# python-graphblas/python-graphblas

Measured on AMD Instinct MI355X. Metric: GTEPS (mxv) on R-MAT scale-24, higher is better.
Workload: dtype f32

## Files before the change

include/grb_mi355x.h:

```cpp
#ifndef GRB_MI355X_H
#define GRB_MI355X_H

#include <stdbool.h>
#include <stddef.h>
#include <stdint.h>

#ifdef __cplusplus
extern "C" {
#endif

#define GRB_VERSION 2
#define GRB_SUBVERSION 0

typedef uint64_t GrB_Index;
#define GrB_INDEX_MAX ((GrB_Index)(1ULL << 60) - 1)

typedef enum {
    GrB_SUCCESS = 0,
    GrB_NO_VALUE = 1,
    GrB_UNINITIALIZED_OBJECT = -1,
    GrB_NULL_POINTER = -2,
    GrB_INVALID_VALUE = -3,
    GrB_INVALID_INDEX = -4,
    GrB_DOMAIN_MISMATCH = -5,
// ... 192 lines not shown
    int64_t flops;
    int64_t out_nvals;
    int32_t method;
    int32_t fused_epilogue;
    int64_t hot_k;
    int64_t long_entries;
    int64_t long_segments;
    int32_t long_kernel;
    int32_t reorders;
    int64_t ordered;
    int64_t value_dict;
    int64_t fill_absent;
    int64_t long_probe;
    int64_t long_tails;
    int64_t pinned_natural;
} GrX_Stats;
GrB_Info GrX_last_stats(GrX_Stats *stats);
GrB_Info GrX_mxm_streamed(const GrB_Semiring semiring, const GrB_Matrix A, const GrB_Matrix B, uint64_t budget_bytes,
                          uint64_t *nvals, uint64_t *checksum, uint64_t *flops, uint64_t *batches);
GrB_Info GrX_Matrix_isclose(bool *result, const GrB_Matrix A, const GrB_Matrix B, double rel_tol, double abs_tol);
GrB_Info GrX_Matrix_dup_as(GrB_Matrix *C, const GrB_Type type, const GrB_Matrix A);
GrB_Info GrX_Vector_dup_as(GrB_Vector *w, const GrB_Type type, const GrB_Vector u);
GrB_Info GrX_Vector_fill_absent(GrB_Vector v, const GrB_Monoid monoid);
GrB_Info GrX_Matrix_cache_bytes(const GrB_Matrix A, uint64_t *bytes);
GrB_Info GrX_option_set(const char *name, int64_t value);
GrB_Info GrX_option_get(const char *name, int64_t *value);
GrB_Info GrX_options_reset(void);
const char *GrX_version_string(void);

#define GRB_DECL_UNARY(T)                                                                                              \
// ... 89 lines not shown
```

python-graphblas_amd/_lib.py:

```python
from __future__ import annotations

import ctypes
import os

_HERE = os.path.dirname(os.path.abspath(__file__))
DEFAULT_LIB = os.path.join(_HERE, "csrc", "libgrb_mi355x.so")

lib = None
_handles = {}

c_void_p = ctypes.c_void_p
c_u64 = ctypes.c_uint64
c_int = ctypes.c_int

TYPE_NAMES = ["BOOL", "INT8", "INT16", "INT32", "INT64", "UINT8", "UINT16", "UINT32", "UINT64", "FP32", "FP64"]

GrB_SUCCESS = 0
GrB_NO_VALUE = 1


class GrX_Stats(ctypes.Structure):
    _fields_ = [("kernel_launches", ctypes.c_int64), ("tiles", ctypes.c_int64), ("flops", ctypes.c_int64),
                ("out_nvals", ctypes.c_int64), ("method", ctypes.c_int32), ("fused_epilogue", ctypes.c_int32),
                ("hot_k", ctypes.c_int64), ("long_entries", ctypes.c_int64), ("long_segments", ctypes.c_int64),
                ("long_kernel", ctypes.c_int32), ("reorders", ctypes.c_int32), ("ordered", ctypes.c_int64), ("value_dict", ctypes.c_int64), ("fill_absent", ctypes.c_int64),
                ("long_probe", ctypes.c_int64), ("long_tails", ctypes.c_int64), ("pinned_natural", ctypes.c_int64)]


def load(path: str | None = None):
    global lib
    if lib is not None:
        return lib
    path = path or os.environ.get("GRB_MI355X_LIB") or DEFAULT_LIB
    if not os.path.exists(path):
        raise ImportError(
            f"{path} not found: build it with `python -c 'import __graft_entry__ as g; g.build()'` "
            "(there is no pure-Python or CPU fallback)"
        )
    if os.path.basename(path) == os.path.basename(DEFAULT_LIB):
        _share_hip_runtime_with_torch()
    lib = ctypes.CDLL(path)
# ... 151 lines not shown
```

python-graphblas_amd/csrc/grb_context.hip:

```cpp
#include <chrono>
#include <algorithm>
#include <cctype>
#include <cstdlib>
#include <cstring>
#include <mutex>
#include <unordered_map>
#include <vector>

#include "grb_internal.hpp"

namespace grb {

#ifdef GRB_ABLATE
static constexpr int DEBUG_FLAGS_MASK = ~0;
#else
static constexpr int DEBUG_FLAGS_MASK = 128 | 256 | 2048 | 65536;
#endif


Context &ctx()
{
    static Context c;
    return c;
}
// ... 183 lines not shown
    int Context::*i;
    int64_t Context::*l;
    enum Rule { ANY, WITHIN, ONE_OF, CLAMP } rule;
    int64_t lo, hi;
    bool (*hook)(int64_t &value);
};
using Hook = bool (*)(int64_t &);
constexpr int64_t MAX64 = INT64_MAX, P30 = 1 << 30;
constexpr Option opt(const char *n, int Context::*f, Option::Rule r = Option::ANY, int64_t lo = 0, int64_t hi = 0, Hook h = nullptr) { return {n, f, nullptr, r, lo, hi, h}; }
constexpr Option opt(const char *n, int64_t Context::*f, Option::Rule r = Option::ANY, int64_t lo = 0, int64_t hi = 0, Hook h = nullptr) { return {n, nullptr, f, r, lo, hi, h}; }

bool known_debug_flags(int64_t &v) { return !((int)v & ~DEBUG_FLAGS_MASK); }
bool short_kernel_exists(int64_t &v) { return v != 2 && v != 3 && v != 4; }
bool snap_long_classes(int64_t &v) { if (v != 16 && v != 32 && v != 64) v = 8; return true; }
bool window_group(int64_t &v) { return (v & (v - 1)) == 0; }
bool release_cache_when_off(int64_t &v) { if (!v) dev_cache_release(); return true; }

const Option OPTIONS[] = {
    opt("debug_flags", &Context::debug_flags, Option::ANY, 0, 0, known_debug_flags),
    opt("pull_ipt", &Context::tune_pull_ipt),
    opt("hot_min_cols", &Context::hot_min_cols),
    opt("hot_k", &Context::hot_k),
    opt("push_mode", &Context::push_mode),
    opt("split_min_nnz", &Context::split_min_nnz),
    opt("split_min_len", &Context::split_min_len, Option::CLAMP, 0, P30),
    opt("short_kernel", &Context::short_kernel, Option::WITHIN, 0, 6, short_kernel_exists),
    opt("lazy_layout", &Context::lazy_layout),
    opt("lazy_min_nnz", &Context::lazy_min_nnz),
    opt("lean_min_nnz", &Context::lean_min_nnz, Option::CLAMP, 0, MAX64),
    opt("long_kernel", &Context::long_kernel),
// ... 10 lines not shown
    opt("mxm_unit_small", &Context::mxm_unit_small, Option::WITHIN, 1, P30),
    opt("mxm_unit_mid", &Context::mxm_unit_mid, Option::WITHIN, 1, P30),
    opt("mxm_unit_dense", &Context::mxm_unit_dense, Option::WITHIN, 1, P30),
    opt("mxm_sym_windows", &Context::mxm_sym_windows, Option::WITHIN, 1, 64),
    opt("mxm_window_groups", &Context::mxm_window_groups, Option::WITHIN, 0, 8, window_group),
    opt("mxm_xcd_map", &Context::mxm_xcd_map, Option::WITHIN, 0, 1),
    opt("mxm_checksum_pass", &Context::mxm_checksum_pass, Option::WITHIN, 0, 1),
    opt("mxm_bitmap_pool_mb", &Context::mxm_bitmap_pool_mb),
    opt("mxm_bitmap_min_cnt", &Context::mxm_bitmap_min_cnt),
    opt("mxm_bitmap_pool_cap", &Context::mxm_bitmap_pool_cap),
    opt("vec_pad_min_bytes", &Context::vec_pad_min_bytes),
    opt("hub_min_len", &Context::hub_min_len, Option::CLAMP, 0, P30),
    opt("fill_absent", &Context::fill_absent, Option::WITHIN, 0, 1),
    opt("rows_tile", &Context::rows_tile, Option::WITHIN, 0, 2),
    opt("lazy_tagged", &Context::lazy_tagged, Option::WITHIN, 0, 1),
    opt("ctile_pack", &Context::ctile_pack, Option::WITHIN, 0, 2),
    opt("strip_slot16", &Context::strip_slot16, Option::WITHIN, 0, 1),
    opt("rtile_pack", &Context::rtile_pack, Option::WITHIN, 0, 1),
    opt("cold_in_rows", &Context::cold_in_rows, Option::CLAMP, 0, P30),
    opt("stream_nt_min_nnz", &Context::stream_nt_min_nnz, Option::CLAMP, 0, MAX64),
    opt("bool_probe", &Context::bool_probe, Option::WITHIN, 0, 16),
    opt("rtile_rows", &Context::rtile_rows, Option::ONE_OF, 8192, 16384),
    opt("rtile_entries", &Context::rtile_entries, Option::WITHIN, 256, 1 << 24),
    opt("rows_head", &Context::rows_head, Option::WITHIN, 0, 1),
    opt("rows_head_min_groups", &Context::rows_head_min_groups, Option::CLAMP, 0, MAX64),
    opt("push_small", &Context::push_small, Option::WITHIN, 0, 1),
    opt("value_dict", &Context::value_dict, Option::WITHIN, 0, 1),
    opt("order_mode", &Context::order_mode, Option::WITHIN, 0, 1),
    opt("order_min_nnz", &Context::order_min_nnz, Option::CLAMP, 0, MAX64),
    opt("alloc_cache", &Context::alloc_cache, Option::ANY, 0, 0, release_cache_when_off),
};
// ... 211 lines not shown
```

python-graphblas_amd/csrc/grb_internal.hpp:

```cpp
#pragma once
#include <hip/hip_runtime.h>

#include <cstdint>
#include <cstdio>
#include <cstring>
#include <memory>
#include <string>
#include <type_traits>

#include "grb_mi355x.h"

namespace grb {

enum TypeCode : int {
    TC_BOOL = 0, TC_INT8, TC_INT16, TC_INT32, TC_INT64, TC_UINT8, TC_UINT16, TC_UINT32, TC_UINT64, TC_FP32, TC_FP64,
    TC_COUNT
};

enum OpCode : int {
    OP_NONE = -1,
    OP_FIRST = 0, OP_SECOND, OP_PAIR, OP_PLUS, OP_MINUS, OP_RMINUS, OP_TIMES, OP_MIN, OP_MAX,
    OP_LOR, OP_LAND, OP_LXOR, OP_LXNOR, OP_ANY, OP_COUNT,
    OP_EQ = 32, OP_NE, OP_GT, OP_LT, OP_GE, OP_LE,
    OP_UNSUPPORTED = 1000
// ... 80 lines not shown
    int rows_head = 1;
    int64_t rows_head_min_groups = 16384;
    int push_small = 1;
    int fill_absent = 1;
    int hub_min_len = 1024;
    int value_dict = 1;
    int order_mode = 1;
    int64_t order_min_nnz = 24ll << 20;
    int64_t reorder_count = 0;
    void *host_stage = nullptr;
    bool host_stage_failed = false;
    void *host_pinned = nullptr;
    unsigned long long *push_counters = nullptr;
    int push_parity = 0;
    int lazy_tagged = 1;
    int ctile_pack = 0;
    int strip_slot16 = 1;
    int rtile_pack = 1;
    int cold_in_rows = 0;
};
Context &ctx();
void require_init();

void *dev_alloc(size_t bytes);
void *dev_alloc_zero(size_t bytes);
void dev_free(void *p);
void dev_cache_release();
void h2d(void *dst, const void *src, size_t bytes);
void d2h(void *dst, const void *src, size_t bytes);
void d2d(void *dst, const void *src, size_t bytes);
// ... 394 lines not shown
```

python-graphblas_amd/csrc/grb_mxv.hip:

```cpp
#include <algorithm>
#include <cstring>
#include <vector>

#include "grb_internal.hpp"
#include "grb_ops.hpp"

namespace grb {

#include "grb_mxv_common.inc"
#include "grb_mxv_pull.inc"
#include "grb_mxv_long.inc"
#include "grb_mxv_vdict.inc"
#include "grb_mxv_strip.inc"
#include "grb_mxv_rows.inc"
#include "grb_mxv_rows_tag.inc"
#include "grb_mxv_ctile.inc"
#include "grb_mxv_rtile.inc"
#include "grb_mxv_split_build.inc"
#include "grb_mxv_write.inc"
#include "grb_mxv_push.inc"
#include "grb_mxv_hot.inc"
#include "grb_mxv_order.inc"

static int64_t hot_table_size(int64_t n, size_t value_bytes)
// ... 276 lines not shown
                               sub, sub_min_len, (unsigned)ncls, kind == 2 ? 1 : 0, 0u, (const int32_t *)nullptr, 0, (int64_t)0, 0u, 0u, (int64_t)0, 0u, (const int64_t *)nullptr);
            const int nvc = ncls + hub_ncls;
            const int n_cr = own_ranges ? A->order.ct_ncr : COLD_CLS * (int)sub;
            const int nvirt = kind == 4 ? nvc + n_cr + (tail_max > 0 ? 1 : 0) : ncls * (int)sub;
            const int hot_cls = 0;
            const unsigned strip_sub = kind == 4 ? 1u : sub;
            if (strips) {
                int vbits = 1;
                while ((1 << vbits) < nvirt) vbits++;
                prim_sort_pairs_u64_u32_bits(keys.p, keys2.p, idx.p, idx2.p, nnz_keyed, 32, 32 + vbits);
            } else {
                prim_sort_pairs_u64_u32(keys.p, keys2.p, idx.p, idx2.p, nnz_keyed, bits);
            }
            int ct_mode = 0;
            std::vector<int32_t> h_bounds;
            if (kind == 4 && own_ranges && ctx().ctile_pack > 0) {
                h_bounds.resize((size_t)A->order.ct_ncr + 1);
                d2h(h_bounds.data(), A->order.d_cold_bounds, sizeof(int32_t) * h_bounds.size());
                int64_t widest = 0;
                for (int r = 0; r < A->order.ct_ncr; r++) widest = std::max<int64_t>(widest, (int64_t)h_bounds[(size_t)r + 1] - (int64_t)h_bounds[(size_t)r]);
                if (widest < ((int64_t)1 << 19) - 1) ct_mode = (ctx().ctile_pack == 2 && A->vd.vdict_n > 0 && A->type->size == 4 && !A->iso) ? 2 : 1;
            }
            const int ct_slots = ct_mode ? CT_PACK_SLOTS : (A->type->size > 4 ? CT_SLOTS / 2 : CT_SLOTS);
            const int n_sb = (int)ceil_div(nl, (int64_t)ct_slots);
            const int64_t n_tiles = kind == 4 ? (int64_t)n_cr * n_sb : 0;
            std::vector<int64_t> h_first((size_t)n_tiles + 1, 0);
            DevBuf<int64_t> tile_first(n_tiles + 1);
            int64_t n_strip = nnz_long;
            if (kind == 4) {
                hipLaunchKernelGGL(k_ctile_first, dim3((unsigned)ceil_div(n_tiles + 1, 256)), dim3(256), 0, ctx().stream, (const uint64_t *)keys2.p, nnz_keyed,
                                   n_tiles, n_sb, (unsigned)nvc, tile_first.p, ct_slots);
                d2h(h_first.data(), tile_first.p, sizeof(int64_t) * (size_t)(n_tiles + 1));
                n_strip = h_first[0];
                if (h_first[(size_t)n_tiles] != nnz_long)
                    fail(GrB_PANIC, "long / short split: the short part and the class keys disagree about the cold entries that moved (internal error)");
            }
            if (kind == 4) {
                sp.long_nnz = nnz_long;
// ... 137 lines not shown
                        sp.strips.d_strip_cb.reset((int64_t *)dev_alloc(sizeof(int64_t) * (size_t)(nvc + 1)));
                        h2d(sp.strips.d_strip_cb, h_cb, sizeof(int64_t) * (size_t)(nvc + 1));
                        sp.strips.wg_tab_g = G;
                    }
                    if (getenv("GRB_PRINT_STRIPS")) {
                        fprintf(stderr, "[strips kind %d] %d classes (%d of them the hub level's), chunks per class:", kind, nvc, hub_ncls);
                        for (int c = 0; c < nvc; c++) fprintf(stderr, " %lld", (long long)(h_cb[c + 1] - h_cb[c]));
                        fprintf(stderr, "  segments %lld\n", (long long)nseg);
                    }
                    sp.strips.strip_ncls = ncls;
                    sp.strips.strip_nseg = nseg;
                    sp.long_nnz = nnz_long;
                    sync_stream();
                }
            }
            const bool use_dict_all = ct_mode == 2;
            if (kind == 4 && nnz_long > n_strip) {
                std::vector<CTile> h_tiles;
                std::vector<int64_t> h_efirst;
                std::vector<int> tile_range;
                std::vector<int64_t> range_cnt((size_t)n_cr, 0);
                int64_t units = 0;
                for (int64_t t = 0; t < n_tiles; t++) {
                    const int64_t cnt = h_first[t + 1] - h_first[t];
                    if (cnt == 0) continue;
                    const int64_t pieces = ceil_div(cnt, CT_MAX_ENTRIES), per = ceil_div(cnt, pieces);
                    for (int64_t q = 0; q < pieces; q++) {
                        const int64_t e0 = h_first[t] + q * per, e1 = std::min<int64_t>(h_first[t] + (q + 1) * per, h_first[t + 1]);
                        CTile ct;
                        ct.u0 = units;
                        ct.n_units = (int32_t)ceil_div(e1 - e0, (int64_t)CT_EPL);
// ... 22 lines not shown
                    }
                } else {
                    for (int r = 0; r < n_cr; r++) range_xcd[(size_t)r] = r % 8;
                }
                std::vector<int32_t> h_order;
                h_order.reserve((size_t)nt);
                for (int x = 0; x < 8; x++) {
                    sp.cold.ct_xoff[x] = (int64_t)h_order.size();
                    for (int64_t t = 0; t < nt; t++)
                        if (range_xcd[(size_t)tile_range[(size_t)t]] == x) h_order.push_back((int32_t)t);
                }
                sp.cold.ct_xoff[8] = (int64_t)h_order.size();
                const size_t ents = (size_t)std::max<int64_t>(units, 1) * CT_EPL;
                sp.cold.d_ct_tiles.reset(dev_alloc((sizeof(CTile) + sizeof(int32_t)) * (size_t)std::max<int64_t>(nt, 1)));
                h2d(sp.cold.d_ct_tiles, h_tiles.data(), sizeof(CTile) * (size_t)nt);
                if (ct_mode) {
                    std::vector<int32_t> h_cbase((size_t)nt);
                    for (int64_t t = 0; t < nt; t++) h_cbase[(size_t)t] = h_bounds[(size_t)tile_range[(size_t)t]];
                    h2d((char *)sp.cold.d_ct_tiles.get() + sizeof(CTile) * (size_t)std::max<int64_t>(nt, 1), h_cbase.data(), sizeof(int32_t) * (size_t)nt);
                }
                sp.cold.d_ct_order.reset((int32_t *)dev_alloc(sizeof(int32_t) * (size_t)std::max<int64_t>(nt, 1)));
                h2d(sp.cold.d_ct_order, h_order.data(), sizeof(int32_t) * (size_t)nt);
                DevBuf<int64_t> efirst(nt + 1);
                h2d(efirst.p, h_efirst.data(), sizeof(int64_t) * (size_t)(nt + 1));
                sp.cold.d_ct_col.reset((int32_t *)dev_alloc(sizeof(int32_t) * ents));
                const size_t ct_vb = use_dict_all ? 1 : A->type->size;
                sp.cold.d_ct_val.reset(A->iso ? nullptr : dev_alloc(ct_vb * ents));
                sp.cold.d_ct_loc.reset(ct_mode ? nullptr : (uint16_t *)dev_alloc(sizeof(uint16_t) * ents));
                GRB_HIP(hipMemsetAsync(sp.cold.d_ct_col, 0xff, sizeof(int32_t) * ents, ctx().stream));
                if (sp.cold.d_ct_val) GRB_HIP(hipMemsetAsync(sp.cold.d_ct_val, 0, ct_vb * ents, ctx().stream));
                if (sp.cold.d_ct_loc) GRB_HIP(hipMemsetAsync(sp.cold.d_ct_loc, 0, sizeof(uint16_t) * ents, ctx().stream));
                const int64_t n_cold = nnz_long - n_strip;
                {
                    DevBuf<uint64_t> key2(n_cold), key2s(n_cold);
                    DevBuf<uint32_t> pay(n_cold), pays(n_cold);
                    hipLaunchKernelGGL(k_ctile_keys2, dim3((unsigned)ceil_div(n_cold, 256)), dim3(256), 0, ctx().stream, (const uint32_t *)idx2.p, n_strip, n_cold,
                                       (const int64_t *)efirst.p, nt, col_src, key2.p, pay.p);
                    int tbits = 1;
                    while (((int64_t)1 << tbits) < nt) tbits++;
                    prim_sort_pairs_u64_u32(key2.p, key2s.p, pay.p, pays.p, n_cold, 32 + tbits);
                    GRB_DISPATCH_TYPE(A->type->code, T, {
                        hipLaunchKernelGGL((k_ctile_place<T>), dim3((unsigned)ceil_div(n_cold, 256)), dim3(256), 0, ctx().stream, (const uint64_t *)keys2.p,
                                           (const uint32_t *)idx2.p, n_strip, n_cold, (const uint64_t *)key2s.p, (const uint32_t *)pays.p, (const int64_t *)efirst.p,
                                           (const CTile *)sp.cold.d_ct_tiles.get(), (const T *)A->d_val, A->iso ? 1 : 0, sp.cold.d_ct_col, (T *)sp.cold.d_ct_val.get(), sp.cold.d_ct_loc,
                                           use_dict_all ? (const unsigned long long *)A->vd.d_vd_table : (const unsigned long long *)nullptr,
                                           use_dict_all ? (const unsigned char *)A->vd.d_vd_codes : (const unsigned char *)nullptr,
                                           ct_mode ? (const int32_t *)((const char *)sp.cold.d_ct_tiles.get() + sizeof(CTile) * (size_t)std::max<int64_t>(nt, 1)) : (const int32_t *)nullptr);
                    })
                    sync_stream();
                }
                sp.cold.ct_mode = ct_mode;
                sp.cold.ct_ntiles = nt;
                sp.cold.ct_units = units;
                if (getenv("GRB_PRINT_STRIPS")) {
                    fprintf(stderr, "[cold tiles] mode %d (slots %d), %d column ranges, %lld tiles, entries per range:", ct_mode, ct_slots, n_cr, (long long)nt);
                    for (int r = 0; r < n_cr; r++) fprintf(stderr, " %lld(x%d)", (long long)range_cnt[(size_t)r], range_xcd[(size_t)r]);
                    fprintf(stderr, "\n");
                }
                sync_stream();
            }
            DevBuf<int64_t> vptr(strips ? 0 : nv + 1), icnt(strips ? 0 : nv + 1);
            if (!strips) {
// ... 67 lines not shown
        if (A->hot_identity) {
            dev_free(A->d_col);
            A->d_col = nullptr;
        } else {
            A->hot.d_col_hot.reset();
        }
        A->hot.hot_cols_dropped = true;
    }
}

static uint64_t order_signature()
{
    const Context &c = ctx();
    uint64_t h = 1469598103934665603ull;
    const int64_t v[] = {c.long_kernel, c.short_kernel, c.long_classes, c.split_min_len, c.long_sub, c.long_sub_min_len, c.lean_min_nnz,
                         c.split_min_nnz, c.hot_k, c.drop_hot_cols, c.hub_min_len, c.value_dict, c.rows_tile, c.rtile_rows, c.rtile_entries, c.cold_in_rows, c.rtile_pack, c.strip_slot16, c.ctile_pack, c.lazy_tagged};
    for (int64_t x : v) h = (h ^ (uint64_t)x) * 1099511628211ull;
    return h;
}

static GB_Perm *ensure_perm(GB_Matrix_opaque *S, int64_t k_hot, DevBuf<unsigned int> &poscnt)
{
    const int64_t n = (int64_t)S->ncols, nnz = S->nvals;
    GB_Matrix_opaque *partner = S->tr ? S->tr : S->tr_of;
    const bool adopt = !S->order.perm && partner && partner->order.perm;
    if (adopt) {
        S->order.perm = partner->order.perm;
        perm_retain(S->order.perm);
    }
    DevBuf<unsigned int> cnt(n, true);
    const int hstride = nnz >= ((int64_t)1 << 26) ? 8 : 1;
// ... 410 lines not shown
            for (int c = 0; c <= A->split.strips.strip_ncls; c++) a.strip_cb[c] = A->split.strips.strip_cb[c];
            a.strip_ncls = A->split.strips.strip_ncls;
            const int64_t G = std::max<int64_t>(A->split.strips.strip_ncls, (int64_t)(ctx().num_cus / A->split.strips.strip_ncls) * A->split.strips.strip_ncls);
            if (A->split.split_kind == 4) {
                a.hrec = A->split.strips.d_hrec;
                a.hrec_bytes = A->split.strips.hrec_bytes;
                a.vdict = A->vd.vdict_n > 0 ? A->vd.d_vdict.get() : nullptr;
                ctx().stats.value_dict = A->vd.vdict_n;
                auto launch_ctile = [&]() {
                    if (A->split.cold.ct_units <= 0) return;
                    a.ct_col = A->split.cold.d_ct_col;
                    a.ct_val = A->split.cold.d_ct_val;
                    a.ct_loc = A->split.cold.d_ct_loc;
                    a.ct_tiles = (const CTile *)A->split.cold.d_ct_tiles.get();
                    a.ct_mode = A->split.cold.ct_mode;
                    a.ct_cbase = A->split.cold.ct_mode ? (const int32_t *)((const char *)A->split.cold.d_ct_tiles.get() + sizeof(CTile) * (size_t)std::max<int64_t>(A->split.cold.ct_ntiles, 1)) : nullptr;
                    if (A->split.cold.ct_mode == 2) a.vdict = A->vd.d_vdict;
                    a.ct_order = A->split.cold.d_ct_order;
                    for (int x = 0; x <= 8; x++) a.ct_xoff[x] = A->split.cold.ct_xoff[x];
                    const int64_t Gt = std::max<int64_t>(8, (int64_t)(ctx().num_cus * CT_WGS_PER_CU / 8) * 8);
                    hipLaunchKernelGGL((k_mxv_ctile<T, MON, MUL>), dim3((unsigned)Gt), dim3(CT_BLOCK), 0, ctx().stream, a);
                    ctx().stats.kernel_launches += 1;
                };
                bool merged = false;
                if constexpr (MON >= 0) {
                    if constexpr (hstrip_fast_semiring<T>(MON, MUL)) {
                        if (hot_fast && A->split.strips.hub_ncls > 0 && A->split.strips.d_wg_tab && A->split.strips.wg_tab_g > 0 && A->split.strips.strip_cb[A->split.strips.strip_ncls + A->split.strips.hub_ncls] > 0) {
                            PullArgs al = a;
                            al.wg_tab = A->split.strips.d_wg_tab;
                            al.strip_cb_dev = A->split.strips.d_strip_cb;
                            al.strip_chunks = A->split.strips.strip_cb[A->split.strips.strip_ncls + A->split.strips.hub_ncls];
                            bool dict_launched = false;
                            const bool s16 = al.strip_slot16 != nullptr;
                            if constexpr (sizeof(T) == 4) {
                                if (al.vdict) {
// ... 282 lines not shown
    DescFlags f;
    if (d) { f.replace = d->replace; f.comp = d->comp; f.structure = d->structure; f.t0 = d->t0; f.t1 = d->t1; }
    return f;
}

static void mxv_core(GB_Vector_opaque *w, GB_Vector_opaque *mask, const GB_BinaryOp_opaque *accum,
                     const GB_Semiring_opaque *sr, GB_Matrix_opaque *S, GB_Vector_opaque *u, bool flip, DescFlags f)
{
    if (S->ncols != u->n) fail(GrB_DIMENSION_MISMATCH, "mxv/vxm: matrix inner dimension " + std::to_string(S->ncols) + " does not match vector size " + std::to_string(u->n));
    if (w->n != S->nrows) fail(GrB_DIMENSION_MISMATCH, "mxv/vxm: output size " + std::to_string(w->n) + " does not match matrix dimension " + std::to_string(S->nrows));
    if (mask && mask->n != w->n) fail(GrB_DIMENSION_MISMATCH, "mxv/vxm: mask size does not match output size");
    if (accum && (accum->type != w->type->code || op_is_comparison(accum->op))) fail(GrB_DOMAIN_MISMATCH, "mxv/vxm: accum operator type must equal the output type");
    ctx().stats = GrX_Stats{};
    ctx().stats.method = 1;
    ctx().stats.long_kernel = -1;
    ctx().stats.flops = S->nvals;
    ctx().stats.out_nvals = -1;
    const int64_t m = (int64_t)w->n;
    if (m == 0) return;
    if (!mask && f.comp) {
        if (f.replace) vector_release_storage(w);
        return;
    }
    const int st = sr->type;
    const int monoid = canonical_op(st, sr->monoid);
    int mult = canonical_op(st, sr->mult);
    if (flip) mult = flip_op(mult);

    DevBuf<uint64_t> mbits_tmp(0);
    const uint64_t *m_bits = nullptr;
// ... 367 lines not shown
    const int need_u = !(mult == OP_PAIR || mult == OP_SECOND);
    if ((need_a && P->type->code != st) || (need_u && u->type->code != st) || w->type->code != st) return -1;
    if (u->n > 0xffffffffull || w->n > 0x7fffffffull || !u->d_val) return -1;
    const int64_t n_in = (int64_t)u->n, n_out = (int64_t)w->n;
    if (ctx().push_mode == 1 && u->nvals >= 0 && u->nvals * 64 >= n_in) return 0;
    if (ctx().push_mode == 1 && u->nvals >= 0 && n_in > 0 && (double)u->nvals * ((double)P->nvals / (double)n_in) * 128.0 > (double)P->nvals) return 0;
    GB_Vector_opaque *vs[3] = {u, w, mask};
    GB_Perm *ord = (u->n == w->n) ? vectors_common_order(vs, 3) : nullptr;
    if (u->n != w->n)
        for (GB_Vector_opaque *v : vs)
            if (v) vector_set_order(v, nullptr);
    ctx().stats = GrX_Stats{};
    ctx().stats.method = 2;
    ctx().stats.out_nvals = -1;
    ctx().stats.long_kernel = -1;
    PushThin a{};
    a.u_bits = u->d_bits;
    a.n_in = n_in;
    a.n_out = n_out;
    a.in_map = ord ? ord->d_inv : nullptr;
    a.out_map = ord ? ord->d_rank : nullptr;
    a.rowptr = matrix_rowptr(P);
    a.col = P->d_col;
    a.aval = P->d_val;
    a.a_iso = P->iso ? 1 : 0;
    a.u_val = u->d_val;
    a.monoid = monoid;
    a.mult = mult;
    a.need_a = need_a;
    a.need_u = need_u;
// ... 370 lines not shown
```

python-graphblas_amd/csrc/grb_mxv_ctile.inc:

```
#ifndef GRB_CT_SLOTS
#define GRB_CT_SLOTS 16384
#endif
#ifndef GRB_CT_BLOCK
#define GRB_CT_BLOCK 1024
#endif
constexpr int CT_SLOTS = GRB_CT_SLOTS;
constexpr int CT_PACK_SLOTS = 8192, CT_PACK_COLBITS = 19;
constexpr int CT_BLOCK = GRB_CT_BLOCK;
constexpr int CT_EPL = 4;
#ifndef GRB_CT_WGS_PER_CU
#define GRB_CT_WGS_PER_CU 2
#endif
constexpr int CT_WGS_PER_CU = GRB_CT_WGS_PER_CU;
#ifndef GRB_CT_ABL
#define GRB_CT_ABL 0
#endif
struct alignas(16) CTile {
    int64_t u0;
    int32_t n_units;
    int32_t base;
};
template <typename W> struct CtSlots { static constexpr int value = sizeof(W) > 4 ? CT_SLOTS / 2 : CT_SLOTS; };

#ifndef GRB_CT_MAX_ENTRIES
// ... 19 lines not shown
    const int64_t c = (int64_t)blockIdx.x * blockDim.x + threadIdx.x;
    if (c >= n_cold) return;
    const int64_t p = p0 + c;
    int64_t lo = 0, hi = n_tiles;
    while (hi - lo > 1) {
        const int64_t mid = (lo + hi) >> 1;
        if (efirst[mid] <= p) lo = mid;
        else hi = mid;
    }
    key2[c] = ((uint64_t)lo << 32) | (uint64_t)(uint32_t)col[sidx[p]];
    pay[c] = (uint32_t)c;
}
template <typename T>
__global__ void k_ctile_place(const uint64_t *skeys, const uint32_t *sidx, int64_t p0, int64_t n_cold, const uint64_t *key2s, const uint32_t *pays,
                              const int64_t *efirst, const CTile *tiles, const T *val, int iso, int32_t *tcol, T *tval, uint16_t *tloc,
                              const unsigned long long *vd_table, const unsigned char *vd_codes, const int32_t *cbase)
{
    const int64_t q = (int64_t)blockIdx.x * blockDim.x + threadIdx.x;
    if (q >= n_cold) return;
    const uint64_t k2 = key2s[q];
    const int64_t t = (int64_t)(k2 >> 32);
    const int64_t p = p0 + (int64_t)pays[q];
    const int64_t slot = (int64_t)(uint32_t)skeys[p];
    const int64_t d = tiles[t].u0 * CT_EPL + (q - (efirst[t] - p0));
    if (cbase) tcol[d] = (int32_t)((((uint32_t)(slot - tiles[t].base)) << CT_PACK_COLBITS) | (((uint32_t)k2 - (uint32_t)cbase[t]) & ((1u << CT_PACK_COLBITS) - 1u)));
    else tcol[d] = (int32_t)(uint32_t)k2;
    bool coded = false;
    if constexpr (sizeof(T) == 4) {
        if (vd_table) {
            ((unsigned char *)tval)[d] = (unsigned char)vdict_code(vd_table, vd_codes, ((const uint32_t *)val)[sidx[p]]);
            coded = true;
        }
    }
    if (!iso && !coded) tval[d] = val[sidx[p]];
    if (tloc) tloc[d] = (uint16_t)(slot - tiles[t].base);
}

template <typename T, int MONOID_CT, int MULT_CT>
__global__ __launch_bounds__(CT_BLOCK) void k_mxv_ctile(const PullArgs a)
{
    using W = typename Widen<T>::type;
    constexpr int EPL = CT_EPL, SLOTS = CtSlots<W>::value;
    __shared__ W s_acc[SLOTS];
    __shared__ uint32_t s_off[SLOTS / 32];
    __shared__ uint32_t s_has[SLOTS / 32];
    __shared__ uint32_t s_dict[sizeof(T) == 4 ? 256 : 1];
    const int monoid = MONOID_CT >= 0 ? MONOID_CT : a.monoid;
    const int mult = MULT_CT >= 0 ? MULT_CT : a.mult;
    const bool need_aval = a.need_aval != 0, need_uval = a.need_uval != 0;
    const bool stage_vals = need_aval && !a.a_iso;
    const bool snt = a.stream_nt != 0;
    const T iso_v = (a.a_iso && need_aval) ? ((const T *)a.aval)[0] : (T)0;
    const __amdgpu_buffer_rsrc_t xval_rs = make_rsrc(a.u_val, a.x_len * (int64_t)sizeof(T));
    const __amdgpu_buffer_rsrc_t xbits_rs = make_rsrc(a.u_bits, a.u_full ? 0 : ((a.x_len + 63) >> 6) * 8);
    const __amdgpu_buffer_rsrc_t xvbits_rs = make_rsrc(a.u_valbits, a.u_valbits ? ((a.x_len + 63) >> 6) * 8 : 0);
    const __amdgpu_buffer_rsrc_t xpv_rs = make_rsrc(a.u_pv, a.u_pv ? ((a.x_len + 15) >> 4) * 4 : 0);
    const int32_t *tcol = a.ct_col;
    const T *tval = (const T *)a.ct_val;
    const uint16_t *tloc = a.ct_loc;
    W *tl = (W *)a.tl_val;
    const W ident = pull_seed<T, W>(a, monoid);
    const int packed = a.ct_mode;
    const int slots_rt = packed ? (CT_PACK_SLOTS < SLOTS ? CT_PACK_SLOTS : SLOTS) : SLOTS;
    if constexpr (sizeof(T) == 4) {
        if (packed == 2) {
            for (int i = threadIdx.x; i < 256; i += CT_BLOCK) s_dict[i] = ((const uint32_t *)a.vdict)[i];
            __syncthreads();
        }
    }
    const int xcd = (int)(blockIdx.x & 7u), li = (int)(blockIdx.x >> 3), nx = (int)(gridDim.x >> 3);
    const int64_t x0 = a.ct_xoff[xcd], x1 = a.ct_xoff[xcd + 1];
    for (int64_t tl_i = x0 + li; tl_i < x1; tl_i += nx) {
        const CTile tile = a.ct_tiles[a.ct_order[tl_i]];
        if (tile.n_units == 0) continue;
        const int cbase = packed ? a.ct_cbase[a.ct_order[tl_i]] : 0;
        const int rows_here = (int)((a.n_long - tile.base < slots_rt) ? a.n_long - tile.base : slots_rt);
        for (int i = threadIdx.x; i < slots_rt; i += CT_BLOCK) s_acc[i] = ident;
        for (int i = threadIdx.x; i < slots_rt / 32; i += CT_BLOCK) {
            s_has[i] = 0u;
            const int64_t wd = ((int64_t)tile.base >> 5) + i;
            s_off[i] = (a.has_mask && (int64_t)i * 32 < rows_here) ? ~a.long_act[wd] : 0u;
        }
        __syncthreads();
        const int64_t u_end = tile.u0 + tile.n_units;
        constexpr int UB = 1;
        for (int64_t ub0 = tile.u0; ub0 < u_end; ub0 += (int64_t)CT_BLOCK * UB) {
            const int64_t ub = ub0 + threadIdx.x;
            int creg[UB][EPL], rk[UB][EPL], cc[UB][EPL];
            T vreg[UB][EPL];
            bool uv[UB];
#pragma unroll
            for (int k = 0; k < UB; k++) {
                const int64_t u = ub + (int64_t)k * CT_BLOCK;
                uv[k] = u < u_end;
                const int64_t e = (uv[k] ? u : u_end - 1) * EPL;
                const uint4 c4 = ptr_stream_x4(tcol + e, snt);
                creg[k][0] = (int)c4.x; creg[k][1] = (int)c4.y; creg[k][2] = (int)c4.z; creg[k][3] = (int)c4.w;
                if (packed) {
#pragma unroll
                    for (int i = 0; i < EPL; i++) {
                        const unsigned w = (unsigned)creg[k][i];
                        rk[k][i] = (int)(w >> CT_PACK_COLBITS);
                        creg[k][i] = w == 0xffffffffu ? -1 : cbase + (int)(w & ((1u << CT_PACK_COLBITS) - 1u));
                        if (w == 0xffffffffu) rk[k][i] = 0;
                    }
                } else {
                    const uint2 l2 = ptr_stream_x2(tloc + e, snt);
                    rk[k][0] = (int)(l2.x & 0xffffu); rk[k][1] = (int)(l2.x >> 16); rk[k][2] = (int)(l2.y & 0xffffu); rk[k][3] = (int)(l2.y >> 16);
                }
                bool vals_done = false;
                if constexpr (sizeof(T) == 4) {
                    if (stage_vals && packed == 2) {
                        const uint32_t cd = ((const uint32_t *)tval)[uv[k] ? u : u_end - 1];
#pragma unroll
                        for (int i = 0; i < EPL; i++) vreg[k][i] = __builtin_bit_cast(T, s_dict[(cd >> (8 * i)) & 0xffu]);
                        vals_done = true;
                    }
                }
                if (vals_done) {
                } else if (stage_vals) {
                    if constexpr (sizeof(T) == 4) {
                        const uint4 v4 = ptr_stream_x4(tval + e, snt);
                        vreg[k][0] = __builtin_bit_cast(T, v4.x); vreg[k][1] = __builtin_bit_cast(T, v4.y);
                        vreg[k][2] = __builtin_bit_cast(T, v4.z); vreg[k][3] = __builtin_bit_cast(T, v4.w);
                    } else {
#pragma unroll
// ... 52 lines not shown
#pragma unroll
                    for (int k = 0; k < UB; k++)
#pragma unroll
                        for (int i = 0; i < EPL; i++) xv[k][i] = vreg[k][i];
                } else {
#pragma unroll
                    for (int k = 0; k < UB; k++)
#pragma unroll
                        for (int i = 0; i < EPL; i++) xv[k][i] = buf_gather<T>(xval_rs, xp[k][i] ? (unsigned)cc[k][i] * (unsigned)sizeof(T) : 0xfffffff8u);
                }
            } else {
#pragma unroll
                for (int k = 0; k < UB; k++)
#pragma unroll
                    for (int i = 0; i < EPL; i++) xv[k][i] = (T)0;
            }
#pragma unroll
            for (int k = 0; k < UB; k++)
#pragma unroll
                for (int i = 0; i < EPL; i++) {
                    if (!xp[k][i]) continue;
                    const int r = rk[k][i];
                    const T prod = apply_binop<T>(mult, need_aval ? vreg[k][i] : (T)0, xv[k][i]);
                    if (GRB_CT_ABL & 4) { if (prod == (T)12345) s_acc[r] = (W)prod; atomicOr(&s_has[r >> 5], 1u << (r & 31)); continue; }
                    if (monoid == OP_ANY) s_acc[r] = (W)prod;
                    else lds_combine<W>(&s_acc[r], (W)prod, monoid);
                    atomicOr(&s_has[r >> 5], 1u << (r & 31));
                }
        }
        __syncthreads();
// ... 13 lines not shown
```

Baseline: 278.4.

## Pack value-dictionary codes into cold-tile column words for f32 mxv

Adds a new default cold-tile mode that stores the 8-bit value-dictionary code in the top byte of each 24-bit column index, so no separate value array is allocated or streamed. The kernel decodes the code and looks up the value in a shared-memory dictionary. Padding slots are pointed at an extra sentinel slot through a new pad kernel. This cuts per-entry memory traffic in the bandwidth-bound cold path, at the cost of limiting columns to 2^24 and only applying to matrices that have a value dictionary.

```diff
diff --git a/include/grb_mi355x.h b/include/grb_mi355x.h
--- a/include/grb_mi355x.h
+++ b/include/grb_mi355x.h
@@ -230,6 +230,7 @@
     int64_t long_probe;
     int64_t long_tails;
     int64_t pinned_natural;
+    int64_t cold_tile_mode;
 } GrX_Stats;
 GrB_Info GrX_last_stats(GrX_Stats *stats);
 GrB_Info GrX_mxm_streamed(const GrB_Semiring semiring, const GrB_Matrix A, const GrB_Matrix B, uint64_t budget_bytes,
diff --git a/python-graphblas_amd/_lib.py b/python-graphblas_amd/_lib.py
--- a/python-graphblas_amd/_lib.py
+++ b/python-graphblas_amd/_lib.py
@@ -24,7 +24,7 @@
                 ("out_nvals", ctypes.c_int64), ("method", ctypes.c_int32), ("fused_epilogue", ctypes.c_int32),
                 ("hot_k", ctypes.c_int64), ("long_entries", ctypes.c_int64), ("long_segments", ctypes.c_int64),
                 ("long_kernel", ctypes.c_int32), ("reorders", ctypes.c_int32), ("ordered", ctypes.c_int64), ("value_dict", ctypes.c_int64), ("fill_absent", ctypes.c_int64),
-                ("long_probe", ctypes.c_int64), ("long_tails", ctypes.c_int64), ("pinned_natural", ctypes.c_int64)]
+                ("long_probe", ctypes.c_int64), ("long_tails", ctypes.c_int64), ("pinned_natural", ctypes.c_int64), ("cold_tile_mode", ctypes.c_int64)]
 
 
 def load(path: str | None = None):
diff --git a/python-graphblas_amd/csrc/grb_context.hip b/python-graphblas_amd/csrc/grb_context.hip
--- a/python-graphblas_amd/csrc/grb_context.hip
+++ b/python-graphblas_amd/csrc/grb_context.hip
@@ -221,6 +221,7 @@
 bool short_kernel_exists(int64_t &v) { return v != 2 && v != 3 && v != 4; }
 bool snap_long_classes(int64_t &v) { if (v != 16 && v != 32 && v != 64) v = 8; return true; }
 bool window_group(int64_t &v) { return (v & (v - 1)) == 0; }
+bool explicit_cold_layout(int64_t &) { ctx().ctile_code = 0; return true; }
 bool release_cache_when_off(int64_t &v) { if (!v) dev_cache_release(); return true; }
 
 const Option OPTIONS[] = {
@@ -261,7 +262,8 @@
     opt("fill_absent", &Context::fill_absent, Option::WITHIN, 0, 1),
     opt("rows_tile", &Context::rows_tile, Option::WITHIN, 0, 2),
     opt("lazy_tagged", &Context::lazy_tagged, Option::WITHIN, 0, 1),
-    opt("ctile_pack", &Context::ctile_pack, Option::WITHIN, 0, 2),
+    opt("ctile_pack", &Context::ctile_pack, Option::WITHIN, 0, 2, explicit_cold_layout),
+    opt("ctile_code", &Context::ctile_code, Option::WITHIN, 0, 1),
     opt("strip_slot16", &Context::strip_slot16, Option::WITHIN, 0, 1),
     opt("rtile_pack", &Context::rtile_pack, Option::WITHIN, 0, 1),
     opt("cold_in_rows", &Context::cold_in_rows, Option::CLAMP, 0, P30),
diff --git a/python-graphblas_amd/csrc/grb_internal.hpp b/python-graphblas_amd/csrc/grb_internal.hpp
--- a/python-graphblas_amd/csrc/grb_internal.hpp
+++ b/python-graphblas_amd/csrc/grb_internal.hpp
@@ -118,6 +118,7 @@
     unsigned long long *push_counters = nullptr;
     int push_parity = 0;
     int lazy_tagged = 1;
+    int ctile_code = 1;
     int ctile_pack = 0;
     int strip_slot16 = 1;
     int rtile_pack = 1;
diff --git a/python-graphblas_amd/csrc/grb_mxv.hip b/python-graphblas_amd/csrc/grb_mxv.hip
--- a/python-graphblas_amd/csrc/grb_mxv.hip
+++ b/python-graphblas_amd/csrc/grb_mxv.hip
@@ -314,6 +314,8 @@
             }
             int ct_mode = 0;
             std::vector<int32_t> h_bounds;
+            if (kind == 4 && ctx().ctile_code == 1 && ctx().ctile_pack == 0 && A->vd.vdict_n > 0 && A->type->size == 4 && A->type->code != TC_BOOL && !A->iso && codes_total <= ((int64_t)1 << 24))
+                ct_mode = 3;
             if (kind == 4 && own_ranges && ctx().ctile_pack > 0) {
                 h_bounds.resize((size_t)A->order.ct_ncr + 1);
                 d2h(h_bounds.data(), A->order.d_cold_bounds, sizeof(int32_t) * h_bounds.size());
@@ -321,7 +323,8 @@
                 for (int r = 0; r < A->order.ct_ncr; r++) widest = std::max<int64_t>(widest, (int64_t)h_bounds[(size_t)r + 1] - (int64_t)h_bounds[(size_t)r]);
                 if (widest < ((int64_t)1 << 19) - 1) ct_mode = (ctx().ctile_pack == 2 && A->vd.vdict_n > 0 && A->type->size == 4 && !A->iso) ? 2 : 1;
             }
-            const int ct_slots = ct_mode ? CT_PACK_SLOTS : (A->type->size > 4 ? CT_SLOTS / 2 : CT_SLOTS);
+            const bool ct_packed = ct_mode == 1 || ct_mode == 2;
+            const int ct_slots = ct_packed ? CT_PACK_SLOTS : (A->type->size > 4 ? CT_SLOTS / 2 : CT_SLOTS);
             const int n_sb = (int)ceil_div(nl, (int64_t)ct_slots);
             const int64_t n_tiles = kind == 4 ? (int64_t)n_cr * n_sb : 0;
             std::vector<int64_t> h_first((size_t)n_tiles + 1, 0);
@@ -489,7 +492,7 @@
                     sync_stream();
                 }
             }
-            const bool use_dict_all = ct_mode == 2;
+            const bool use_dict_all = ct_mode == 2 || ct_mode == 3;
             if (kind == 4 && nnz_long > n_strip) {
                 std::vector<CTile> h_tiles;
                 std::vector<int64_t> h_efirst;
@@ -542,7 +545,7 @@
                 const size_t ents = (size_t)std::max<int64_t>(units, 1) * CT_EPL;
                 sp.cold.d_ct_tiles.reset(dev_alloc((sizeof(CTile) + sizeof(int32_t)) * (size_t)std::max<int64_t>(nt, 1)));
                 h2d(sp.cold.d_ct_tiles, h_tiles.data(), sizeof(CTile) * (size_t)nt);
-                if (ct_mode) {
+                if (ct_packed) {
                     std::vector<int32_t> h_cbase((size_t)nt);
                     for (int64_t t = 0; t < nt; t++) h_cbase[(size_t)t] = h_bounds[(size_t)tile_range[(size_t)t]];
                     h2d((char *)sp.cold.d_ct_tiles.get() + sizeof(CTile) * (size_t)std::max<int64_t>(nt, 1), h_cbase.data(), sizeof(int32_t) * (size_t)nt);
@@ -553,11 +556,14 @@
                 h2d(efirst.p, h_efirst.data(), sizeof(int64_t) * (size_t)(nt + 1));
                 sp.cold.d_ct_col.reset((int32_t *)dev_alloc(sizeof(int32_t) * ents));
                 const size_t ct_vb = use_dict_all ? 1 : A->type->size;
-                sp.cold.d_ct_val.reset(A->iso ? nullptr : dev_alloc(ct_vb * ents));
-                sp.cold.d_ct_loc.reset(ct_mode ? nullptr : (uint16_t *)dev_alloc(sizeof(uint16_t) * ents));
+                sp.cold.d_ct_val.reset((A->iso || ct_mode == 3) ? nullptr : dev_alloc(ct_vb * ents));
+                sp.cold.d_ct_loc.reset(ct_packed ? nullptr : (uint16_t *)dev_alloc(sizeof(uint16_t) * ents));
                 GRB_HIP(hipMemsetAsync(sp.cold.d_ct_col, 0xff, sizeof(int32_t) * ents, ctx().stream));
                 if (sp.cold.d_ct_val) GRB_HIP(hipMemsetAsync(sp.cold.d_ct_val, 0, ct_vb * ents, ctx().stream));
                 if (sp.cold.d_ct_loc) GRB_HIP(hipMemsetAsync(sp.cold.d_ct_loc, 0, sizeof(uint16_t) * ents, ctx().stream));
+                if (ct_mode == 3 && nt > 0)
+                    hipLaunchKernelGGL(k_ctile_pad_slots, dim3((unsigned)ceil_div(nt, 256)), dim3(256), 0, ctx().stream, (const CTile *)sp.cold.d_ct_tiles.get(),
+                                       (const int64_t *)efirst.p, nt, sp.cold.d_ct_loc.get(), (uint16_t)ct_slots);
                 const int64_t n_cold = nnz_long - n_strip;
                 {
                     DevBuf<uint64_t> key2(n_cold), key2s(n_cold);
@@ -573,7 +579,8 @@
                                            (const CTile *)sp.cold.d_ct_tiles.get(), (const T *)A->d_val, A->iso ? 1 : 0, sp.cold.d_ct_col, (T *)sp.cold.d_ct_val.get(), sp.cold.d_ct_loc,
                                            use_dict_all ? (const unsigned long long *)A->vd.d_vd_table : (const unsigned long long *)nullptr,
                                            use_dict_all ? (const unsigned char *)A->vd.d_vd_codes : (const unsigned char *)nullptr,
-                                           ct_mode ? (const int32_t *)((const char *)sp.cold.d_ct_tiles.get() + sizeof(CTile) * (size_t)std::max<int64_t>(nt, 1)) : (const int32_t *)nullptr);
+                                           ct_packed ? (const int32_t *)((const char *)sp.cold.d_ct_tiles.get() + sizeof(CTile) * (size_t)std::max<int64_t>(nt, 1)) : (const int32_t *)nullptr,
+                                           ct_mode == 3 ? 1 : 0);
                     })
                     sync_stream();
                 }
@@ -671,7 +678,7 @@
     const Context &c = ctx();
     uint64_t h = 1469598103934665603ull;
     const int64_t v[] = {c.long_kernel, c.short_kernel, c.long_classes, c.split_min_len, c.long_sub, c.long_sub_min_len, c.lean_min_nnz,
-                         c.split_min_nnz, c.hot_k, c.drop_hot_cols, c.hub_min_len, c.value_dict, c.rows_tile, c.rtile_rows, c.rtile_entries, c.cold_in_rows, c.rtile_pack, c.strip_slot16, c.ctile_pack, c.lazy_tagged};
+                         c.split_min_nnz, c.hot_k, c.drop_hot_cols, c.hub_min_len, c.value_dict, c.rows_tile, c.rtile_rows, c.rtile_entries, c.cold_in_rows, c.rtile_pack, c.strip_slot16, c.ctile_pack, c.ctile_code, c.lazy_tagged};
     for (int64_t x : v) h = (h ^ (uint64_t)x) * 1099511628211ull;
     return h;
 }
@@ -1112,11 +1119,19 @@
                     a.ct_loc = A->split.cold.d_ct_loc;
                     a.ct_tiles = (const CTile *)A->split.cold.d_ct_tiles.get();
                     a.ct_mode = A->split.cold.ct_mode;
-                    a.ct_cbase = A->split.cold.ct_mode ? (const int32_t *)((const char *)A->split.cold.d_ct_tiles.get() + sizeof(CTile) * (size_t)std::max<int64_t>(A->split.cold.ct_ntiles, 1)) : nullptr;
-                    if (A->split.cold.ct_mode == 2) a.vdict = A->vd.d_vdict;
+                    const int ctm = A->split.cold.ct_mode;
+                    a.ct_cbase = (ctm == 1 || ctm == 2) ? (const int32_t *)((const char *)A->split.cold.d_ct_tiles.get() + sizeof(CTile) * (size_t)std::max<int64_t>(A->split.cold.ct_ntiles, 1)) : nullptr;
+                    if (ctm == 2 || ctm == 3) a.vdict = A->vd.d_vdict;
+                    ctx().stats.cold_tile_mode = ctm;
                     a.ct_order = A->split.cold.d_ct_order;
                     for (int x = 0; x <= 8; x++) a.ct_xoff[x] = A->split.cold.ct_xoff[x];
                     const int64_t Gt = std::max<int64_t>(8, (int64_t)(ctx().num_cus * CT_WGS_PER_CU / 8) * 8);
+                    if (ctm == 3) {
+                        if constexpr (sizeof(T) == 4 && !std::is_same<T, bool>::value)
+                            hipLaunchKernelGGL((k_mxv_ctile<T, MON, MUL, true>), dim3((unsigned)Gt), dim3(CT_BLOCK), 0, ctx().stream, a);
+                        else
+                            fail(GrB_PANIC, "cold tiles: code words built for a type that has no kernel for them (internal error)");
+                    } else
                     hipLaunchKernelGGL((k_mxv_ctile<T, MON, MUL>), dim3((unsigned)Gt), dim3(CT_BLOCK), 0, ctx().stream, a);
                     ctx().stats.kernel_launches += 1;
                 };
@@ -1429,6 +1444,7 @@
     ctx().stats = GrX_Stats{};
     ctx().stats.method = 1;
     ctx().stats.long_kernel = -1;
+    ctx().stats.cold_tile_mode = -1;
     ctx().stats.flops = S->nvals;
     ctx().stats.out_nvals = -1;
     const int64_t m = (int64_t)w->n;
@@ -1826,6 +1842,7 @@
     ctx().stats.method = 2;
     ctx().stats.out_nvals = -1;
     ctx().stats.long_kernel = -1;
+    ctx().stats.cold_tile_mode = -1;
     PushThin a{};
     a.u_bits = u->d_bits;
     a.n_in = n_in;
diff --git a/python-graphblas_amd/csrc/grb_mxv_ctile.inc b/python-graphblas_amd/csrc/grb_mxv_ctile.inc
--- a/python-graphblas_amd/csrc/grb_mxv_ctile.inc
+++ b/python-graphblas_amd/csrc/grb_mxv_ctile.inc
@@ -57,7 +57,7 @@
 template <typename T>
 __global__ void k_ctile_place(const uint64_t *skeys, const uint32_t *sidx, int64_t p0, int64_t n_cold, const uint64_t *key2s, const uint32_t *pays,
                               const int64_t *efirst, const CTile *tiles, const T *val, int iso, int32_t *tcol, T *tval, uint16_t *tloc,
-                              const unsigned long long *vd_table, const unsigned char *vd_codes, const int32_t *cbase)
+                              const unsigned long long *vd_table, const unsigned char *vd_codes, const int32_t *cbase, int code_word)
 {
     const int64_t q = (int64_t)blockIdx.x * blockDim.x + threadIdx.x;
     if (q >= n_cold) return;
@@ -71,7 +71,9 @@
     bool coded = false;
     if constexpr (sizeof(T) == 4) {
         if (vd_table) {
-            ((unsigned char *)tval)[d] = (unsigned char)vdict_code(vd_table, vd_codes, ((const uint32_t *)val)[sidx[p]]);
+            const uint32_t code = (uint32_t)vdict_code(vd_table, vd_codes, ((const uint32_t *)val)[sidx[p]]) & 0xffu;
+            if (code_word) tcol[d] = (int32_t)((code << 24) | ((uint32_t)k2 & 0x00ffffffu));
+            else ((unsigned char *)tval)[d] = (unsigned char)code;
             coded = true;
         }
     }
@@ -79,13 +81,22 @@
     if (tloc) tloc[d] = (uint16_t)(slot - tiles[t].base);
 }
 
-template <typename T, int MONOID_CT, int MULT_CT>
+__global__ void k_ctile_pad_slots(const CTile *tiles, const int64_t *efirst, int64_t n_tiles, uint16_t *tloc, uint16_t pad_slot)
+{
+    const int64_t t = (int64_t)blockIdx.x * blockDim.x + threadIdx.x;
+    if (t >= n_tiles) return;
+    const int64_t d0 = tiles[t].u0 * CT_EPL, d1 = d0 + (int64_t)tiles[t].n_units * CT_EPL;
+    for (int64_t d = d0 + (efirst[t + 1] - efirst[t]); d < d1; d++) tloc[d] = pad_slot;
+}
+
+template <typename T, int MONOID_CT, int MULT_CT, bool CODEW = false>
 __global__ __launch_bounds__(CT_BLOCK) void k_mxv_ctile(const PullArgs a)
 {
     using W = typename Widen<T>::type;
     constexpr int EPL = CT_EPL, SLOTS = CtSlots<W>::value;
+    static_assert(!CODEW || (sizeof(T) == 4 && !std::is_same<T, bool>::value && SLOTS == CT_SLOTS), "code words: 4-byte values, tiles of CT_SLOTS slots");
     __shared__ W s_acc[SLOTS];
-    __shared__ uint32_t s_off[SLOTS / 32];
+    __shared__ uint32_t s_off[SLOTS / 32 + (CODEW ? 1 : 0)];
     __shared__ uint32_t s_has[SLOTS / 32];
     __shared__ uint32_t s_dict[sizeof(T) == 4 ? 256 : 1];
     const int monoid = MONOID_CT >= 0 ? MONOID_CT : a.monoid;
@@ -103,9 +114,12 @@
     const uint16_t *tloc = a.ct_loc;
     W *tl = (W *)a.tl_val;
     const W ident = pull_seed<T, W>(a, monoid);
-    const int packed = a.ct_mode;
+    const int packed = CODEW ? 0 : a.ct_mode;
     const int slots_rt = packed ? (CT_PACK_SLOTS < SLOTS ? CT_PACK_SLOTS : SLOTS) : SLOTS;
-    if constexpr (sizeof(T) == 4) {
+    if constexpr (CODEW) {
+        for (int i = threadIdx.x; i < 256; i += CT_BLOCK) s_dict[i] = ((const uint32_t *)a.vdict)[i];
+        if (threadIdx.x == 0) s_off[SLOTS / 32] = ~0u;
+    } else if constexpr (sizeof(T) == 4) {
         if (packed == 2) {
             for (int i = threadIdx.x; i < 256; i += CT_BLOCK) s_dict[i] = ((const uint32_t *)a.vdict)[i];
             __syncthreads();
@@ -131,6 +145,7 @@
             const int64_t ub = ub0 + threadIdx.x;
             int creg[UB][EPL], rk[UB][EPL], cc[UB][EPL];
             T vreg[UB][EPL];
+            unsigned vcode[UB][EPL];
             bool uv[UB];
 #pragma unroll
             for (int k = 0; k < UB; k++) {
@@ -139,7 +154,16 @@
                 const int64_t e = (uv[k] ? u : u_end - 1) * EPL;
                 const uint4 c4 = ptr_stream_x4(tcol + e, snt);
                 creg[k][0] = (int)c4.x; creg[k][1] = (int)c4.y; creg[k][2] = (int)c4.z; creg[k][3] = (int)c4.w;
-                if (packed) {
+                if constexpr (CODEW) {
+                    const uint2 l2 = ptr_stream_x2(tloc + e, snt);
+                    rk[k][0] = (int)(l2.x & 0xffffu); rk[k][1] = (int)(l2.x >> 16); rk[k][2] = (int)(l2.y & 0xffffu); rk[k][3] = (int)(l2.y >> 16);
+#pragma unroll
+                    for (int i = 0; i < EPL; i++) {
+                        const unsigned w = (unsigned)creg[k][i];
+                        creg[k][i] = (int)(w & 0x00ffffffu);
+                        vcode[k][i] = w >> 24;
+                    }
+                } else if (packed) {
 #pragma unroll
                     for (int i = 0; i < EPL; i++) {
                         const unsigned w = (unsigned)creg[k][i];
@@ -151,8 +175,8 @@
                     const uint2 l2 = ptr_stream_x2(tloc + e, snt);
                     rk[k][0] = (int)(l2.x & 0xffffu); rk[k][1] = (int)(l2.x >> 16); rk[k][2] = (int)(l2.y & 0xffffu); rk[k][3] = (int)(l2.y >> 16);
                 }
-                bool vals_done = false;
-                if constexpr (sizeof(T) == 4) {
+                bool vals_done = CODEW;
+                if constexpr (sizeof(T) == 4 && !CODEW) {
                     if (stage_vals && packed == 2) {
                         const uint32_t cd = ((const uint32_t *)tval)[uv[k] ? u : u_end - 1];
 #pragma unroll
@@ -235,6 +259,12 @@
                 for (int k = 0; k < UB; k++)
 #pragma unroll
                     for (int i = 0; i < EPL; i++) xv[k][i] = (T)0;
+            }
+            if constexpr (CODEW) {
+#pragma unroll
+                for (int k = 0; k < UB; k++)
+#pragma unroll
+                    for (int i = 0; i < EPL; i++) vreg[k][i] = stage_vals ? __builtin_bit_cast(T, s_dict[vcode[k][i]]) : iso_v;
             }
 #pragma unroll
             for (int k = 0; k < UB; k++)
```

New measurement: 291.3, median of 6. 1.05x the previous value.
